# apache/cassandra

Measured on NVIDIA H100. Metric: compaction MB/s (uncompressed in), higher is better.
Workload: dtype u8

## Files before the change

### cassandra_b200/csrc/codec.cuh

```cuda
#pragma once
#include "common.cuh"
#include "lz4.cuh"
#include "lz4_chain.cuh"
#include "snappy_chain.cuh"
#include "snappy.cuh"
#include "codec_defs.cuh"
#include "lz4_thread.cuh"
#include "lz4_batch.cuh"

namespace b200c {

__global__ void __launch_bounds__(32) k_compress_chunks(const DevTables* __restrict__ T, int comp, int tab_bytes,
        const uint8_t* __restrict__ in, uint64_t n, int chunk_len, int max_clen,
        uint8_t* __restrict__ slots, int slot_stride, uint32_t* __restrict__ file_len, uint32_t* __restrict__ seg_raw) {
    extern __shared__ __align__(16) uint8_t smem[];
    uint16_t* s_tab = (uint16_t*)smem;
    uint8_t* s_in = smem + tab_bytes;
    const int lane = threadIdx.x;
    const uint64_t chunk = blockIdx.x;
    const uint64_t start = chunk * (uint64_t)chunk_len;
    const int ulen = (int)min((uint64_t)chunk_len, n - start);
    const uint8_t* src = in + start;

    if ((((uintptr_t)src) & 15) == 0) {
// ... 38 lines not shown

template <bool DUP>
__global__ void __launch_bounds__(32) k_compress_chunks_lz4_direct(const DevTables* __restrict__ T,
        const uint8_t* __restrict__ in, uint64_t n, int chunk_len, int max_clen,
        uint8_t* __restrict__ slots, int slot_stride, uint32_t* __restrict__ file_len, uint32_t* __restrict__ seg_raw) {
    __shared__ __align__(16) uint16_t s_tab[LZ4_TABLE_ENTRIES];
    __shared__ uint8_t s_dup[DUP ? LZ4_DUP_ENTRIES : 1];
    const int lane = threadIdx.x;
    const uint64_t chunk = blockIdx.x;
    const uint64_t start = chunk * (uint64_t)chunk_len;
    const int ulen = (int)min((uint64_t)chunk_len, n - start);
    const uint8_t* src = in + start;
    uint8_t* slot = slots + chunk * (uint64_t)slot_stride;
    if (lane == 0) { slot[0] = (uint8_t)ulen; slot[1] = (uint8_t)(ulen >> 8); slot[2] = (uint8_t)(ulen >> 16); slot[3] = (uint8_t)(ulen >> 24); }
    int clen = 4 + lz4_compress_warp<true>(src, ulen, s_tab, slot + 4, lane, DUP ? s_dup : nullptr);
    if (clen >= max_clen) {
        for (int i = lane; i < ulen; i += 32) slot[i] = src[i];
        clen = ulen;
        if (ulen < max_clen) { for (int i = ulen + lane; i < max_clen; i += 32) slot[i] = 0; clen = max_clen; }
    }
    __syncwarp();
    __threadfence_block();
    uint32_t raw = warp_crc32_raw(T, T->crc_adv128, slot, clen, lane);
    uint32_t init = gf2_mulmod(0xFFFFFFFFu, warp_xpow8n(T, (uint32_t)clen, lane));
    uint32_t crc = ~(raw ^ init);
    if (lane == 0) {
        slot[clen] = (uint8_t)(crc >> 24); slot[clen + 1] = (uint8_t)(crc >> 16); slot[clen + 2] = (uint8_t)(crc >> 8); slot[clen + 3] = (uint8_t)crc;
        file_len[chunk] = (uint32_t)clen + 4;
        uint32_t x = raw ^ __byte_perm(crc, 0, 0x0123);
        seg_raw[chunk] = T->crc_t[3][x & 0xff] ^ T->crc_t[2][(x >> 8) & 0xff] ^ T->crc_t[1][(x >> 16) & 0xff] ^ T->crc_t[0][x >> 24];
    }
}

__global__ void __launch_bounds__(32) k_lz4_chain_build(const uint8_t* __restrict__ in, uint64_t n, int chunk_len, uint32_t* __restrict__ ent) {
    __shared__ __align__(16) uint16_t s_t1[LZ4_TABLE_ENTRIES];
    const uint64_t start = (uint64_t)blockIdx.x * (uint64_t)chunk_len;
    const int ulen = (int)min((uint64_t)chunk_len, n - start);
    lz4_chain_build_warp<true>(in + start, ulen, s_t1, ent + start, threadIdx.x);
}
enum { K5B_WARPS = 4 };
__global__ void __launch_bounds__(32 * K5B_WARPS) k_compress_chunks_lz4_chain(const DevTables* __restrict__ T,
        const uint8_t* __restrict__ in, uint64_t n, int chunk_len, int max_clen, const uint32_t* __restrict__ ent,
        uint8_t* __restrict__ slots, int slot_stride, uint32_t* __restrict__ file_len, uint32_t* __restrict__ seg_raw, uint64_t nchunks) {
    extern __shared__ __align__(16) uint32_t s_bits[];
    const int lane = threadIdx.x & 31, wid = threadIdx.x >> 5;
    const uint64_t chunk = (uint64_t)blockIdx.x * K5B_WARPS + wid;
    if (chunk >= nchunks) return;
    const uint64_t start = chunk * (uint64_t)chunk_len;
    const int ulen = (int)min((uint64_t)chunk_len, n - start);
    const uint8_t* src = in + start;
    uint8_t* slot = slots + chunk * (uint64_t)slot_stride;
    if (lane == 0) { slot[0] = (uint8_t)ulen; slot[1] = (uint8_t)(ulen >> 8); slot[2] = (uint8_t)(ulen >> 16); slot[3] = (uint8_t)(ulen >> 24); }
    int clen = 4 + lz4_compress_warp_chain(src, ulen, ent + start, s_bits + (size_t)wid * ((chunk_len + 31) >> 5), slot + 4, lane);
    if (clen >= max_clen) {
        for (int i = lane; i < ulen; i += 32) slot[i] = src[i];
        clen = ulen;
        if (ulen < max_clen) { for (int i = ulen + lane; i < max_clen; i += 32) slot[i] = 0; clen = max_clen; }
    }
    __syncwarp();
    __threadfence_block();
    uint32_t raw = warp_crc32_raw(T, T->crc_adv128, slot, clen, lane);
    uint32_t init = gf2_mulmod(0xFFFFFFFFu, warp_xpow8n(T, (uint32_t)clen, lane));
    uint32_t crc = ~(raw ^ init);
    if (lane == 0) {
        slot[clen] = (uint8_t)(crc >> 24); slot[clen + 1] = (uint8_t)(crc >> 16); slot[clen + 2] = (uint8_t)(crc >> 8); slot[clen + 3] = (uint8_t)crc;
        file_len[chunk] = (uint32_t)clen + 4;
        uint32_t x = raw ^ __byte_perm(crc, 0, 0x0123);
        seg_raw[chunk] = T->crc_t[3][x & 0xff] ^ T->crc_t[2][(x >> 8) & 0xff] ^ T->crc_t[1][(x >> 16) & 0xff] ^ T->crc_t[0][x >> 24];
    }
}

__global__ void __launch_bounds__(32) k_snappy_chain_build(int max_bits, int table_size, const uint8_t* __restrict__ in, uint64_t n, int chunk_len, uint32_t* __restrict__ ent) {
    extern __shared__ __align__(16) uint8_t smem_sc[];
    const uint64_t start = (uint64_t)blockIdx.x * (uint64_t)chunk_len;
    const int ulen = (int)min((uint64_t)chunk_len, n - start);
    snappy_chain_build_warp<true>(in + start, ulen, max_bits, (uint16_t*)smem_sc, ent + start, threadIdx.x);
}
__global__ void __launch_bounds__(32 * K5B_WARPS) k_compress_chunks_snappy_chain(const DevTables* __restrict__ T,
        const uint8_t* __restrict__ in, uint64_t n, int chunk_len, int max_clen, const uint32_t* __restrict__ ent,
        uint8_t* __restrict__ slots, int slot_stride, uint32_t* __restrict__ file_len, uint32_t* __restrict__ seg_raw, uint64_t nchunks) {
    extern __shared__ __align__(16) uint32_t s_bits[];
    const int lane = threadIdx.x & 31, wid = threadIdx.x >> 5;
    const uint64_t chunk = (uint64_t)blockIdx.x * K5B_WARPS + wid;
    if (chunk >= nchunks) return;
    const uint64_t start = chunk * (uint64_t)chunk_len;
    const int ulen = (int)min((uint64_t)chunk_len, n - start);
    const uint8_t* src = in + start;
    uint8_t* slot = slots + chunk * (uint64_t)slot_stride;
    int clen = snappy_compress_warp_chain(src, ulen, ent + start, s_bits + (size_t)wid * ((chunk_len + 31) >> 5), slot, lane);
    if (clen >= max_clen) {
        for (int i = lane; i < ulen; i += 32) slot[i] = src[i];
        clen = ulen;
        if (ulen < max_clen) { for (int i = ulen + lane; i < max_clen; i += 32) slot[i] = 0; clen = max_clen; }
    }
    __syncwarp();
    __threadfence_block();
    uint32_t raw = warp_crc32_raw(T, T->crc_adv128, slot, clen, lane);
    uint32_t init = gf2_mulmod(0xFFFFFFFFu, warp_xpow8n(T, (uint32_t)clen, lane));
    uint32_t crc = ~(raw ^ init);
    if (lane == 0) {
        slot[clen] = (uint8_t)(crc >> 24); slot[clen + 1] = (uint8_t)(crc >> 16); slot[clen + 2] = (uint8_t)(crc >> 8); slot[clen + 3] = (uint8_t)crc;
        file_len[chunk] = (uint32_t)clen + 4;
        uint32_t x = raw ^ __byte_perm(crc, 0, 0x0123);
        seg_raw[chunk] = T->crc_t[3][x & 0xff] ^ T->crc_t[2][(x >> 8) & 0xff] ^ T->crc_t[1][(x >> 16) & 0xff] ^ T->crc_t[0][x >> 24];
    }
}

__global__ void __launch_bounds__(32) k_compress_chunks_snappy_direct(const DevTables* __restrict__ T, int max_bits,
        const uint8_t* __restrict__ in, uint64_t n, int chunk_len, int max_clen,
        uint8_t* __restrict__ slots, int slot_stride, uint32_t* __restrict__ file_len, uint32_t* __restrict__ seg_raw) {
// ... 254 lines not shown
```

### cassandra_b200/csrc/engine.cu

```cuda
#include "engine.cuh"
#include <algorithm>
#include "scan.cuh"
#include "codec.cuh"
#include <climits>
#include <vector>

using namespace b200c;

namespace b200c {

enum { WSC_IN = 0, WSC_OUT, WSC_SLOTS, WSC_FILELEN, WSC_SEGRAW, WSC_OFFS, WSC_ACC, WSC_ERR, WSC_CHOFFS, WSC_SCAN0, WSC_SCAN1, WSC_SCAN2 };

static void build_tables(DevTables* t) {
    for (uint32_t i = 0; i < 256; i++) {
        uint32_t c = i;
        for (int k = 0; k < 8; k++) c = (c & 1) ? (0xEDB88320u ^ (c >> 1)) : (c >> 1);
        t->crc_t[0][i] = c;
    }
    for (uint32_t i = 0; i < 256; i++)
        for (int k = 1; k < 4; k++) t->crc_t[k][i] = (t->crc_t[k - 1][i] >> 8) ^ t->crc_t[0][t->crc_t[k - 1][i] & 0xff];
    uint32_t sq = 0x00800000u;
    for (int k = 0; k < 64; k++) { t->xp_pow2[k] = sq; sq = gf2_mulmod(sq, sq); }
    auto xpow8n = [&](uint64_t n) { uint32_t r = 0x80000000u; for (int k = 0; n; k++, n >>= 1) if (n & 1) r = gf2_mulmod(r, t->xp_pow2[k]); return r; };
    uint32_t x128 = xpow8n(128);
    for (int j = 0; j < 4; j++)
        for (uint32_t b = 0; b < 256; b++) t->crc_adv128[j][b] = gf2_mulmod(b << (8 * j), x128);
    for (int l = 0; l < 32; l++) t->xp_lane[l] = xpow8n(4 * (32 - l));
}

template <typename TIn>
int exclusive_scan(b200c_ctx* c, const TIn* in, uint64_t n, uint64_t* out, int slot, int depth) {
    if (n == 0) { B200C_CUDA_TRY(c, cudaMemsetAsync(out, 0, sizeof(uint64_t), c->stream)); return B200C_OK; }
    uint64_t tiles = (n + SCAN_TILE - 1) / SCAN_TILE;
    if (tiles == 1) { B200C_LAUNCH(c, k_scan_down<TIn>, 1, SCAN_THREADS, 0, in, n, (const uint64_t*)nullptr, out, out + n); return B200C_OK; }
    if (depth > 2) { c->err = "scan recursion too deep"; return B200C_EINVAL; }
    uint64_t* sums; B200C_TRY(ws_typed(c, slot + depth, tiles + 1, &sums));
    B200C_LAUNCH(c, k_scan_reduce<TIn>, (unsigned)tiles, SCAN_THREADS, 0, in, n, sums);
    B200C_TRY(exclusive_scan<uint64_t>(c, sums, tiles, sums, slot, depth + 1));
    B200C_LAUNCH(c, k_scan_down<TIn>, (unsigned)tiles, SCAN_THREADS, 0, in, n, (const uint64_t*)sums, out, out + n);
    return B200C_OK;
}
template int exclusive_scan<uint32_t>(b200c_ctx*, const uint32_t*, uint64_t, uint64_t*, int, int);
template int exclusive_scan<uint64_t>(b200c_ctx*, const uint64_t*, uint64_t, uint64_t*, int, int);

int compress_slots_device(b200c_ctx* c, int comp, const uint8_t* d_in, uint64_t n, int chunk_len, int max_clen,
                          uint8_t* slots, int stride, uint32_t* file_len, uint32_t* seg_raw) {
    uint64_t nchunks = (n + chunk_len - 1) / chunk_len;
    if (!nchunks) return B200C_OK;
    const int k5_env = []() { const char* e = getenv("B200C_K5"); return e ? atoi(e) : -1; }();
    const int k5_mode = k5_env >= 0 ? k5_env : (comp_is_snappy(comp) ? 3 : 1);
    if (k5_mode == 3 && comp == COMP_LZ4 && ((uintptr_t)d_in & 3) == 0 && (chunk_len & 3) == 0 && chunk_len <= LZ4C_MAX_CHUNK) {
        uint32_t* ent; B200C_TRY(ws_typed(c, WS_K5_ENT, (size_t)n + 16384, &ent));
        B200C_LAUNCH(c, k_lz4_chain_build, (unsigned)nchunks, 32, 0, d_in, n, chunk_len, ent);
        const size_t smem = (size_t)K5B_WARPS * ((chunk_len + 31) >> 5) * 4;
        B200C_LAUNCH(c, k_compress_chunks_lz4_chain, (unsigned)((nchunks + K5B_WARPS - 1) / K5B_WARPS), 32 * K5B_WARPS, smem, c->d_tables, d_in, n, chunk_len, max_clen, (const uint32_t*)ent,
                     slots, stride, file_len, seg_raw, nchunks);
        return B200C_OK;
    }
    if ((k5_mode == 1 || k5_mode == 2) && comp == COMP_LZ4 && ((uintptr_t)d_in & 3) == 0 && (chunk_len & 3) == 0) {
        if (k5_mode == 2) B200C_LAUNCH(c, k_compress_chunks_lz4_direct<true>, (unsigned)nchunks, 32, 0, c->d_tables, d_in, n, chunk_len, max_clen, slots, stride, file_len, seg_raw);
        else B200C_LAUNCH(c, k_compress_chunks_lz4_direct<false>, (unsigned)nchunks, 32, 0, c->d_tables, d_in, n, chunk_len, max_clen, slots, stride, file_len, seg_raw);
        return B200C_OK;
    }
    if (k5_mode == 3 && comp_is_snappy(comp) && ((uintptr_t)d_in & 3) == 0 && (chunk_len & 3) == 0 && chunk_len <= LZ4C_MAX_CHUNK) {
        const int max_bits = comp == COMP_SNAPPY15 ? 15 : 14, tsz = snappy_table_size(chunk_len, max_bits);
        uint32_t* ent; B200C_TRY(ws_typed(c, WS_K5_ENT, (size_t)n + 16384, &ent));
        static bool attr = false; if (!attr) { cudaFuncSetAttribute(k_snappy_chain_build, cudaFuncAttributeMaxDynamicSharedMemorySize, 2 * 32768); attr = true; }
        B200C_LAUNCH(c, k_snappy_chain_build, (unsigned)nchunks, 32, (size_t)2 * tsz, max_bits, tsz, d_in, n, chunk_len, ent);
        const size_t smem = (size_t)K5B_WARPS * ((chunk_len + 31) >> 5) * 4;
        B200C_LAUNCH(c, k_compress_chunks_snappy_chain, (unsigned)((nchunks + K5B_WARPS - 1) / K5B_WARPS), 32 * K5B_WARPS, smem, c->d_tables, d_in, n, chunk_len, max_clen, (const uint32_t*)ent,
                     slots, stride, file_len, seg_raw, nchunks);
        return B200C_OK;
    }
    int tab_bytes = comp == COMP_SNAPPY15 ? 65536 : (comp == COMP_SNAPPY ? 32768 : 16384);
    if (k5_mode != 0 && comp_is_snappy(comp) && ((uintptr_t)d_in & 3) == 0 && (chunk_len & 3) == 0 && chunk_len <= 65536) {
        int need = 512; while (need < 2 * chunk_len && need < tab_bytes) need <<= 1;
        B200C_LAUNCH(c, k_compress_chunks_snappy_direct, (unsigned)nchunks, 32, (size_t)need, c->d_tables, comp == COMP_SNAPPY15 ? 15 : 14, d_in, n, chunk_len, max_clen, slots, stride, file_len, seg_raw);
        return B200C_OK;
    }
    size_t smem = (size_t)tab_bytes + chunk_len + 16;
    B200C_LAUNCH(c, k_compress_chunks, (unsigned)nchunks, 32, smem, c->d_tables, comp, tab_bytes, d_in, n, chunk_len, max_clen, slots, stride, file_len, seg_raw);
    return B200C_OK;
}
int pack_digest_device(b200c_ctx* c, const uint8_t* slots, int stride, const uint32_t* file_len, const uint32_t* seg_raw, uint64_t nchunks,
                       uint8_t* d_out, uint64_t out_cap, uint64_t* d_offs, uint64_t* out_len, uint32_t* digest, int ws_base) {
    if (!nchunks) { *out_len = 0; *digest = 0; B200C_CUDA_TRY(c, cudaMemsetAsync(d_offs, 0, 8, c->stream)); return B200C_OK; }
    uint32_t* acc; B200C_TRY(ws_typed(c, ws_base + WSC_ACC, 4, &acc));
    B200C_CUDA_TRY(c, cudaMemsetAsync(acc, 0, 16, c->stream));
    B200C_TRY(exclusive_scan<uint32_t>(c, file_len, nchunks, d_offs, ws_base + WSC_SCAN0, 0));
    uint64_t* h = (uint64_t*)c->h_pinned;
    B200C_CUDA_TRY(c, cudaMemcpyAsync(h, d_offs + nchunks, 8, cudaMemcpyDeviceToHost, c->stream));
    B200C_CUDA_TRY(c, cudaStreamSynchronize(c->stream));
    *out_len = h[0];
    if (h[0] > out_cap) { c->err = "output buffer too small"; return B200C_ETOOSMALL; }
    B200C_LAUNCH(c, k_pack_chunks, (unsigned)((nchunks + 3) / 4), 128, 0, slots, stride, file_len, d_offs, nchunks, d_out, (const uint64_t*)nullptr);
    B200C_LAUNCH(c, k_digest, (unsigned)((nchunks + 255) / 256), 256, 0, c->d_tables, seg_raw, d_offs, nchunks, acc);
    B200C_LAUNCH(c, k_digest_final, 1, 1, 0, c->d_tables, d_offs, nchunks, acc);
    uint32_t* h32 = (uint32_t*)c->h_pinned;
    B200C_CUDA_TRY(c, cudaMemcpyAsync(h32, acc + 1, 4, cudaMemcpyDeviceToHost, c->stream));
    B200C_CUDA_TRY(c, cudaStreamSynchronize(c->stream));
    *digest = h32[0];
    return B200C_OK;
}
int compress_stream_device(b200c_ctx* c, int comp, const uint8_t* d_in, uint64_t n, int chunk_len, int max_clen,
                           uint8_t* d_out, uint64_t out_cap, uint64_t* d_offs , uint64_t* out_len, uint32_t* digest, int ws_base) {
    uint64_t nchunks = (n + chunk_len - 1) / chunk_len;
    if (nchunks > 0x7fffffffull) { c->err = "too many chunks"; return B200C_EINVAL; }
    int stride = chunk_slot_stride(comp, chunk_len);
// ... 148 lines not shown

int b200c_abi_version(void) { return B200C_ABI_VERSION; }

int b200c_device_count(void) {
    int n = 0; if (cudaGetDeviceCount(&n) != cudaSuccess) { cudaGetLastError(); return 0; } return n;
}

b200c_ctx* b200c_create(int device, size_t workspace_bytes) {
    int n = b200c_device_count();
    if (device < 0 || device >= n) return nullptr;
    if (cudaSetDevice(device) != cudaSuccess) return nullptr;
    b200c_ctx* c = new b200c_ctx();
    c->device = device;
    if (cudaDeviceGetAttribute(&c->nsm, cudaDevAttrMultiProcessorCount, device) != cudaSuccess || c->nsm <= 0) { delete c; return nullptr; }
    if (cudaDeviceGetAttribute(&c->l2_bytes, cudaDevAttrL2CacheSize, device) != cudaSuccess || c->l2_bytes <= 0) { delete c; return nullptr; }
    if (cudaDeviceGetAttribute(&c->smem_per_sm, cudaDevAttrMaxSharedMemoryPerMultiprocessor, device) != cudaSuccess ||
        cudaDeviceGetAttribute(&c->smem_reserved_per_block, cudaDevAttrReservedSharedMemoryPerBlock, device) != cudaSuccess) { delete c; return nullptr; }
    if (cudaStreamCreateWithFlags(&c->stream, cudaStreamNonBlocking) != cudaSuccess) { delete c; return nullptr; }
    cudaEventCreate(&c->ev0); cudaEventCreate(&c->ev1);
    for (auto& e : c->ev_stage) cudaEventCreate(&e);
    cudaStreamCreateWithFlags(&c->copy_stream, cudaStreamNonBlocking);
    for (auto& e : c->ev_in) cudaEventCreateWithFlags(&e, cudaEventDisableTiming);
    for (auto& e : c->ev_pool) cudaEventCreateWithFlags(&e, cudaEventDisableTiming);
    cudaStreamCreateWithFlags(&c->copy_out, cudaStreamNonBlocking);
    cudaStreamCreateWithFlags(&c->stream5, cudaStreamNonBlocking);
    DevTables* h = new DevTables(); build_tables(h);
    if (cudaMalloc(&c->d_tables, sizeof(DevTables)) != cudaSuccess) { delete h; delete c; return nullptr; }
    cudaMemcpy(c->d_tables, h, sizeof(DevTables), cudaMemcpyHostToDevice);
    delete h;
    c->h_pinned_cap = 1 << 16;
    if (cudaMallocHost(&c->h_pinned, c->h_pinned_cap) != cudaSuccess) { cudaFree(c->d_tables); delete c; return nullptr; }
    cudaFuncSetAttribute(k_compress_chunks, cudaFuncAttributeMaxDynamicSharedMemorySize, 65536 + 65536 + 16);
    cudaFuncSetAttribute(k_compress_chunks_snappy_direct, cudaFuncAttributeMaxDynamicSharedMemorySize, 65536);
    k1_plan(c);
    (void)workspace_bytes;
    return c;
}

void b200c_destroy(b200c_ctx* c) {
    if (!c) return;
    cudaSetDevice(c->device);
    cudaStreamSynchronize(c->stream);
    for (auto& b : c->ws) if (b.p) cudaFree(b.p);
    if (c->d_tables) cudaFree(c->d_tables);
    if (c->h_pinned) cudaFreeHost(c->h_pinned);
    cudaEventDestroy(c->ev0); cudaEventDestroy(c->ev1);
    for (auto& e : c->ev_stage) cudaEventDestroy(e);
    for (auto& e : c->ev_in) cudaEventDestroy(e);
    for (auto& e : c->ev_pool) cudaEventDestroy(e);
    for (auto& e : c->ev_marks) cudaEventDestroy(e);
    if (c->stream5) cudaStreamDestroy(c->stream5);
    for (auto e : c->ev_k5) cudaEventDestroy(e);
    if (c->copy_out) cudaStreamDestroy(c->copy_out);
    if (c->copy_stream) cudaStreamDestroy(c->copy_stream);
    cudaStreamDestroy(c->stream);
    delete c;
}

const char* b200c_last_error(b200c_ctx* c) { return c ? c->err.c_str() : "no context (no CUDA device?)"; }

int b200c_host_register(void* p, size_t n) { cudaError_t e = cudaHostRegister(p, n, cudaHostRegisterDefault); if (e != cudaSuccess) { cudaGetLastError(); return B200C_ECUDA; } return B200C_OK; }
int b200c_host_unregister(void* p) { cudaError_t e = cudaHostUnregister(p); if (e != cudaSuccess) { cudaGetLastError(); return B200C_ECUDA; } return B200C_OK; }

int b200c_dev_alloc(b200c_ctx* c, size_t n, void** dptr) {
    if (!c || !dptr) return B200C_EINVAL;
    cudaSetDevice(c->device);
// ... 25 lines not shown
uint64_t b200c_chunk_count(uint64_t n, int chunk_len) { return chunk_len > 0 ? (n + chunk_len - 1) / chunk_len : 0; }
uint64_t b200c_compress_bound(int comp, uint64_t n, int chunk_len) {
    uint64_t nch = b200c_chunk_count(n, chunk_len);
    int m = chunk_max_compressed(comp, chunk_len); if (m < chunk_len) m = chunk_len;
    return nch * ((uint64_t)m + 4) + 64;
}
int b200c_initial_compressed_buffer_length(int comp, int chunk_len) { return chunk_max_compressed(comp, chunk_len); }

static int check_codec_args(b200c_ctx* c, int comp, int chunk_len) {
    if (!c) return B200C_EINVAL;
    if (comp != COMP_LZ4 && !comp_is_snappy(comp) && comp != COMP_NONE) { c->err = "unknown compressor"; return B200C_EINVAL; }
    if (chunk_len <= 0 || chunk_len > 65536 || (chunk_len & (chunk_len - 1))) { c->err = "chunk_len must be a power of two <= 64 KiB"; return B200C_EUNSUPPORTED; }
    return B200C_OK;
}

int b200c_compress_chunks(b200c_ctx* c, int comp, const uint8_t* in, uint64_t n, int chunk_len, int max_clen,
                          uint8_t* out, uint64_t out_cap, uint64_t* out_len, uint64_t* chunk_offsets, uint32_t* digest, int flags) {
    B200C_TRY(check_codec_args(c, comp, chunk_len));
    if ((!in && n) || !out || !out_len || !digest) { c->err = "null argument"; return B200C_EINVAL; }
    cudaSetDevice(c->device);
    const bool dev = flags & B200C_FLAG_DEVICE_PTRS;
    uint64_t nchunks = b200c_chunk_count(n, chunk_len);
    const uint8_t* d_in = in; uint8_t* d_out = out; uint64_t* d_offs;
    if (!dev) {
        uint8_t* p; B200C_TRY(ws_typed(c, WSC_IN, n + 64, &p));
        B200C_CUDA_TRY(c, cudaMemcpyAsync(p, in, n, cudaMemcpyHostToDevice, c->stream)); d_in = p;
        B200C_TRY(ws_typed(c, WSC_OUT, out_cap, &d_out));
    }
    if (dev && chunk_offsets) d_offs = chunk_offsets;
    else B200C_TRY(ws_typed(c, WSC_OFFS, nchunks + 1, &d_offs));
    timing_begin(c);
    int rc = compress_stream_device(c, comp, d_in, n, chunk_len, max_clen, d_out, out_cap, d_offs, out_len, digest, 0);
    int rc2 = timing_end(c);
    if (rc != B200C_OK) return rc;
    if (rc2 != B200C_OK) return rc2;
    if (!dev) {
        B200C_CUDA_TRY(c, cudaMemcpyAsync(out, d_out, *out_len, cudaMemcpyDeviceToHost, c->stream));
        if (chunk_offsets && nchunks) B200C_CUDA_TRY(c, cudaMemcpyAsync(chunk_offsets, d_offs, nchunks * 8, cudaMemcpyDeviceToHost, c->stream));
        B200C_CUDA_TRY(c, cudaStreamSynchronize(c->stream));
    }
    return B200C_OK;
}

int b200c_decompress_chunks(b200c_ctx* c, int comp, const uint8_t* data, uint64_t data_len, const uint64_t* chunk_offsets, uint64_t nchunks,
                            int chunk_len, int max_clen, uint64_t data_length, uint8_t* out, int verify_crc, b200c_corruption* where, int flags) {
    B200C_TRY(check_codec_args(c, comp, chunk_len));
    if ((!data && data_len) || (!chunk_offsets && nchunks) || (!out && data_length)) { c->err = "null argument"; return B200C_EINVAL; }
    if (nchunks != b200c_chunk_count(data_length, chunk_len)) { c->err = "chunk count does not match data_length"; return B200C_EINVAL; }
    cudaSetDevice(c->device);
    const bool dev = flags & B200C_FLAG_DEVICE_PTRS;
    const uint8_t* d_data = data; const uint64_t* d_offs = chunk_offsets; uint8_t* d_out = out;
    if (!dev) {
        uint8_t* p; B200C_TRY(ws_typed(c, WSC_IN, data_len + 64, &p));
        B200C_CUDA_TRY(c, cudaMemcpyAsync(p, data, data_len, cudaMemcpyHostToDevice, c->stream)); d_data = p;
        uint64_t* po; B200C_TRY(ws_typed(c, WSC_CHOFFS, nchunks + 1, &po));
        B200C_CUDA_TRY(c, cudaMemcpyAsync(po, chunk_offsets, nchunks * 8, cudaMemcpyHostToDevice, c->stream)); d_offs = po;
        B200C_TRY(ws_typed(c, WSC_OUT, data_length + 64, &d_out));
    }
    ChunkErr* d_err; B200C_TRY(ws_typed(c, WSC_ERR, 1, &d_err));
    B200C_CUDA_TRY(c, cudaMemsetAsync(d_err, 0xFF, sizeof(ChunkErr), c->stream));
    timing_begin(c);
    int rc = decompress_stream_device(c, comp, d_data, data_len, d_offs, nchunks, chunk_len, max_clen, data_length, d_out, verify_crc, d_err, 0, ~0ull, 0, nullptr, ~0ull);
    int rc2 = timing_end(c);
    if (rc != B200C_OK) return rc;
    if (rc2 != B200C_OK) return rc2;
    ChunkErr* h = (ChunkErr*)c->h_pinned;
// ... 53 lines not shown
```

### cassandra_b200/csrc/engine.cuh

```cuda
#pragma once
#include <cstdio>
#include <cstring>
#include <string>
#include <atomic>
#include <chrono>
#include <vector>
#include "../../include/b200c.h"
#include "common.cuh"

namespace b200c {

enum { WS_SLOTS = 160, WS_K5_ENT = 150, WS_K1_REC = 151, WS_K1_NSEQ = 152 };

struct WsBuf { void* p = nullptr; size_t cap = 0; };

}

struct b200c_ctx {
    int device = 0;
    int nsm = 0;
    int l2_bytes = 0;
    int smem_per_sm = 0, smem_reserved_per_block = 0;
    int k1_blocks_per_sm = 1; size_t k1_smem = 0;
    cudaStream_t stream = nullptr;
// ... 19 lines not shown
    std::vector<cudaEvent_t> ev_marks;
    cudaEvent_t ev_pool[256] = {};
    cudaStream_t copy_out = nullptr;
    cudaStream_t stream5 = nullptr;
    std::vector<cudaEvent_t> ev_k5;
};

namespace b200c {

#define B200C_CUDA_TRY(ctx, expr) do { cudaError_t _e = (expr); if (_e != cudaSuccess) { \
    (ctx)->err = std::string(#expr) + ": " + cudaGetErrorString(_e); return B200C_ECUDA; } } while (0)

#define B200C_LAUNCH(ctx, kernel, grid, block, smem, ...) do { \
    kernel<<<(grid), (block), (smem), (ctx)->stream>>>(__VA_ARGS__); \
    (ctx)->launches_call++; (ctx)->launches_total++; \
    cudaError_t _e = cudaGetLastError(); if (_e != cudaSuccess) { \
        (ctx)->err = std::string(#kernel) + " launch: " + cudaGetErrorString(_e); return B200C_ECUDA; } } while (0)

#define B200C_TRY(expr) do { int _rc = (expr); if (_rc != B200C_OK) return _rc; } while (0)

inline int ws_get(b200c_ctx* c, int slot, size_t bytes, void** out) {
    WsBuf& b = c->ws[slot];
    size_t need = bytes + 256;
    if (b.cap < need) {
        if (b.p) { cudaStreamSynchronize(c->stream); if (c->copy_stream) cudaStreamSynchronize(c->copy_stream); if (c->copy_out) cudaStreamSynchronize(c->copy_out); cudaFree(b.p); b.p = nullptr; b.cap = 0; }
        size_t cap = need + need / 8;
        cudaError_t e = cudaMalloc(&b.p, cap);
        if (e != cudaSuccess) { cudaGetLastError(); c->err = "cudaMalloc(" + std::to_string(cap) + "): " + cudaGetErrorString(e); b.p = nullptr; return B200C_ENOMEM; }
        b.cap = cap;
    }
    *out = b.p;
    return B200C_OK;
}
template <typename T> inline int ws_typed(b200c_ctx* c, int slot, size_t count, T** out) {
    void* p; int rc = ws_get(c, slot, count * sizeof(T), &p); *out = (T*)p; return rc;
}

template <typename T> inline int ws_grow_keep(b200c_ctx* c, int slot, size_t count, size_t used, T** out) {
    WsBuf& b = c->ws[slot];
    size_t need = count * sizeof(T) + 256;
    if (b.cap < need) {
        cudaStreamSynchronize(c->stream); cudaStreamSynchronize(c->copy_out);
        void* np = nullptr; size_t cap = need * 2;
        cudaError_t e = cudaMalloc(&np, cap);
        if (e != cudaSuccess) { cudaGetLastError(); c->err = "cudaMalloc(" + std::to_string(cap) + "): " + cudaGetErrorString(e); return B200C_ENOMEM; }
        if (b.p && used) cudaMemcpy(np, b.p, std::min(used * sizeof(T), b.cap), cudaMemcpyDeviceToDevice);
        if (b.p) cudaFree(b.p);
        b.p = np; b.cap = cap;
    }
    *out = (T*)b.p;
    return B200C_OK;
}

inline void timing_begin(b200c_ctx* c) { c->launches_call = 0; cudaEventRecord(c->ev0, c->stream); c->timing = true; }
inline int timing_end(b200c_ctx* c) {
    cudaEventRecord(c->ev1, c->stream);
    B200C_CUDA_TRY(c, cudaEventSynchronize(c->ev1));
    float ms = 0; cudaEventElapsedTime(&ms, c->ev0, c->ev1); c->last_ms = ms; c->timing = false;
    return B200C_OK;
}

struct OutStream {
    enum { MAX_PIECES = 96 };
    b200c_ctx* c = nullptr; int comp = 0, L = 0, max_clen = 0, stride = 0, ws_base = 0;
    uint8_t* h_out = nullptr; uint64_t h_cap = 0;
    uint32_t *file_len = nullptr, *seg_raw = nullptr, *acc = nullptr; uint64_t *d_offs = nullptr, *bases = nullptr;
// ... 11 lines not shown
```

### cassandra_b200/csrc/lz4_chain.cuh

```cuda
#pragma once
#include "lz4.cuh"

namespace b200c {

enum { LZ4C_MAX_CHUNK = 32768, LZ4C_NONE = 0xFFFF, LZ4C_DUP_ENTRIES = 8192 };

#if defined(__CUDA_ARCH__)
#define LZ4C_PREFETCH(p) asm volatile("prefetch.global.L2 [%0];" :: "l"(p))
#else
#define LZ4C_PREFETCH(p) ((void)0)
#endif

__host__ __device__ __forceinline__ int lz4c_positions(int n) { return n >= LZ4_MINLENGTH ? n - LZ4_MFLIMIT + 1 : 0; }

template <bool GLOBAL, class HASH> __device__ __forceinline__ void chain_build_warp(const uint8_t* s_in, int npos, int nent, int hbits, HASH hash, uint16_t* s_t1, uint32_t* __restrict__ ent, int lane) {
    const uint32_t* in32 = (const uint32_t*)s_in;
    {
        uint4* a = (uint4*)s_t1;
        for (int i = lane; i < (nent * 2) / 16; i += 32) a[i] = make_uint4(~0u, ~0u, ~0u, ~0u);
    }
    __syncwarp();
    const uint32_t lt_mask = (1u << lane) - 1u;
    enum { AHEAD = 4 };
    uint32_t ring[AHEAD];
#pragma unroll
    for (int k = 0; k < AHEAD; k++) ring[k] = (32 * k + lane < npos) ? lz4_rd32<GLOBAL>(in32, 32 * k + lane) : 0u;
    for (int p0 = 0; p0 < npos; p0 += 32 * AHEAD) {
#pragma unroll
        for (int k = 0; k < AHEAD; k++) {
            const int p = p0 + 32 * k + lane; const bool valid = p < npos;
            if (p0 + 32 * k >= npos) break;
            const uint32_t seq = ring[k];
            ring[k] = (p + 32 * AHEAD < npos) ? lz4_rd32<GLOBAL>(in32, p + 32 * AHEAD) : 0u;
            const uint32_t h = hash(seq);
            uint32_t q1 = valid ? (uint32_t)s_t1[h] : (uint32_t)LZ4C_NONE;
            __syncwarp();
            if (valid) s_t1[h] = (uint16_t)p;
            __syncwarp();
            const bool lost = valid && s_t1[h] != (uint16_t)p;
            uint32_t todo = __ballot_sync(FULL_MASK, lost);
            if (todo) {
                bool fix = false;
                while (todo) {
                    const int l = __ffs(todo) - 1;
                    const uint32_t hh = __shfl_sync(FULL_MASK, h, l);
                    const uint32_t same = __ballot_sync(FULL_MASK, valid && h == hh);
                    if (valid && h == hh) {
                        const uint32_t lower = same & lt_mask;
                        if (lower) q1 = (uint32_t)(p0 + 32 * k + 31 - __clz(lower));
                        fix = !(same & ~lt_mask & ~(1u << lane));
                    }
                    todo &= ~same;
                }
                if (fix) s_t1[h] = (uint16_t)p;
                __syncwarp();
            }
            if (valid) ent[p] = q1 == LZ4C_NONE ? 0u : q1;
        }
    }
    __syncwarp();
#pragma unroll 8
    for (int p0 = 0; p0 < npos; p0 += 32) {
        const int p = p0 + lane;
        if (p < npos) {
            const uint32_t a1 = ent[p] & 0x7FFFu;
            const uint32_t a2 = ent[a1] & 0x7FFFu;
            const uint32_t sp = lz4_rd32<GLOBAL>(in32, p);
            const uint32_t e1 = lz4_rd32<GLOBAL>(in32, (int)a1) == sp, e2 = lz4_rd32<GLOBAL>(in32, (int)a2) == sp;
            ent[p] = a1 | (e1 << 15) | (a2 << 16) | (e2 << 31);
        }
    }
}
struct Lz4Hash { __device__ __forceinline__ uint32_t operator()(uint32_t seq) const { return lz4_hash_u16(seq); } };
template <bool GLOBAL> __device__ __forceinline__ void lz4_chain_build_warp(const uint8_t* s_in, int n, uint16_t* s_t1, uint32_t* __restrict__ ent, int lane) {
    chain_build_warp<GLOBAL>(s_in, lz4c_positions(n), LZ4_TABLE_ENTRIES, LZ4_HASHLOG_U16, Lz4Hash(), s_t1, ent, lane);
}

__device__ __forceinline__ uint32_t lz4c_range_bits(int lo, int hi, int w) {
    const int a = lo > w * 32 ? lo - w * 32 : 0, b = hi < w * 32 + 32 ? hi - w * 32 : 32;
    if (b <= a) return 0u;
    const uint32_t upto_b = b >= 32 ? FULL_MASK : ((1u << b) - 1u);
    return upto_b & ~((1u << a) - 1u);
}

__device__ int lz4_compress_warp_chain(const uint8_t* s_in, int n, const uint32_t* __restrict__ ent, uint32_t* s_bm, uint8_t* out, int lane) {
    const uint32_t* in32 = (const uint32_t*)s_in;
    for (int i = lane; i < ((n + 31) >> 5); i += 32) s_bm[i] = (i == 0) ? 1u : 0u;
    __syncwarp();
    int anchor = 0, op = 0;
    const int mfl1 = n - LZ4_MFLIMIT + 1;
    const int matchlimit = n - LZ4_LASTLITERALS;

    if (n >= LZ4_MINLENGTH) {
        int fwd = 1; bool have_prefix = false; int pre_ip = 0;
        for (;;) {
            int ip = 0, match = 0, token_pos; bool ended = false, immediate = false;
            if (lane < 4) LZ4C_PREFETCH(ent + fwd + 64 + 32 * lane);
            int a0 = 0;
            for (bool first = true;; first = false) {
                const bool prefixed = first && have_prefix;
                const bool contiguous = a0 + 32 <= 66;
                const int w_lo = prefixed ? pre_ip - 2 : fwd + a0;
                const int hole = prefixed ? pre_ip - 1 : -1;
                int p; bool valid, putonly = false;
                if (contiguous) {
                    p = w_lo + lane + ((prefixed && lane >= 1) ? 1 : 0);
                    putonly = prefixed && lane == 0;
                    valid = (prefixed && lane < 2) || p + 1 <= mfl1;
// ... 127 lines not shown
```

### cassandra_b200/csrc/snappy_chain.cuh

```cuda
#pragma once
#include "snappy.cuh"
#include "lz4_chain.cuh"

namespace b200c {

struct SnappyHash { uint32_t tmask; int max_bits; __device__ __forceinline__ uint32_t operator()(uint32_t bytes) const { return snappy_tidx(bytes, tmask, max_bits); } };
__host__ __device__ __forceinline__ int snappy_table_size(int frag, int max_bits) { int t = 256; while (t < frag && t < (1 << max_bits)) t <<= 1; return t; }
__host__ __device__ __forceinline__ int snappyc_positions(int n) { return n >= 15 ? n - 14 : 0; }

template <bool GLOBAL> __device__ __forceinline__ void snappy_chain_build_warp(const uint8_t* s_in, int n, int max_bits, uint16_t* s_t1, uint32_t* __restrict__ ent, int lane) {
    const int tsz = snappy_table_size(n, max_bits);
    chain_build_warp<GLOBAL>(s_in, snappyc_positions(n), tsz, 31 - __clz(tsz), SnappyHash{(uint32_t)tsz - 1u, max_bits}, s_t1, ent, lane);
}

__device__ int snappy_compress_warp_chain(const uint8_t* s_in, int n, const uint32_t* __restrict__ ent, uint32_t* s_bm, uint8_t* out, int lane) {
    const uint32_t* in32 = (const uint32_t*)s_in;
    int op = 0;
    {   uint32_t v = (uint32_t)n; uint8_t pre[5]; int k = 0;
        while (v >= 0x80) { pre[k++] = (uint8_t)(v | 0x80); v >>= 7; } pre[k++] = (uint8_t)v;
        if (lane == 0) for (int i = 0; i < k; i++) out[i] = pre[i];
        op = k; }
    for (int i = lane; i < ((n + 31) >> 5); i += 32) s_bm[i] = (i == 0) ? 1u : 0u;
    __syncwarp();
    int ip = 0; const int ip_end = n;
    if (n >= 15) {
        const int ip_limit = n - 15;
        bool have_prefix = false;
        for (;;) {
            const int next_emit = ip;
            const int start = ip + 1;
            const bool unrolled = ip_limit - start >= 16;
            int hit_ip = 0, candidate = 0; bool ended = false, immediate = false;
            if (lane < 4) LZ4C_PREFETCH(ent + start + 64 + 32 * lane);
            int q0 = start; uint32_t skip0 = 32; int a0 = 0;
            for (bool first = true;; first = false) {
                const bool prefixed = first && have_prefix;
                const bool contiguous = first;
                const int w_lo = prefixed ? ip - 1 : start;
                int q; bool valid, putonly = false; int qn = 0; uint32_t skn = 0;
                if (contiguous) {
                    q = w_lo + lane;
                    const int l = lane - (prefixed ? 2 : 0);
                    putonly = prefixed && lane == 0;
                    qn = q + 1; skn = 32u + (uint32_t)(l + 1);
                    valid = l < 0 || (unrolled && l < 16) || qn <= ip_limit;
// ... 87 lines not shown
```

Measured before the change: 32330.

## Build hash chain links with block-wide radix sort instead of per-warp scan

Replaces the single-warp sequential hash-chain build with a 512-thread-per-chunk kernel. It loads the chunk into shared memory, stably radix-sorts positions by hash in two digit passes, and derives each position's previous same-hash link from its sorted neighbour. The chain path becomes the default for LZ4 as well as snappy. The kernel uses more shared memory and more synchronisation, and the old warp builder is kept only as a serial lane-0 fallback. A large link workspace is also freed after each call when it exceeds a threshold, which adds a stream synchronize.

After: 32620, median of 6. Within noise of the previous version (+0.9%).

```diff
diff --git a/cassandra_b200/csrc/codec.cuh b/cassandra_b200/csrc/codec.cuh
--- a/cassandra_b200/csrc/codec.cuh
+++ b/cassandra_b200/csrc/codec.cuh
@@ -94,11 +94,117 @@
     }
 }
 
-__global__ void __launch_bounds__(32) k_lz4_chain_build(const uint8_t* __restrict__ in, uint64_t n, int chunk_len, uint32_t* __restrict__ ent) {
-    __shared__ __align__(16) uint16_t s_t1[LZ4_TABLE_ENTRIES];
+enum { LINK_THREADS = 512, LINK_WARPS = LINK_THREADS / 32, LINK_DIGIT_BITS = 8, LINK_DIGITS = 1 << LINK_DIGIT_BITS };
+__host__ __device__ __forceinline__ size_t link_smem_bytes(int chunk_len) {
+    return (size_t)((chunk_len + 16 + 15) & ~15) + (size_t)LINK_WARPS * (LINK_DIGITS + LINK_DIGITS / 2) * 4 + (size_t)2 * 2 * chunk_len;
+}
+struct Lz4Links {
+    Lz4Hash hash; int bits, npos;
+    __device__ Lz4Links(int n, int) : bits(LZ4_HASHLOG_U16), npos(lz4c_positions(n)) {}
+};
+struct SnappyLinks {
+    SnappyHash hash; int bits, npos;
+    __device__ SnappyLinks(int n, int max_bits) {
+        const int tsz = snappy_table_size(n, max_bits);
+        hash = SnappyHash{(uint32_t)tsz - 1u, max_bits}; bits = 31 - __clz(tsz); npos = snappyc_positions(n);
+    }
+};
+__device__ __forceinline__ void link_scan(uint32_t* a, int len, uint32_t* s_wsum) {
+    const int tid = threadIdx.x, lane = tid & 31, w = tid >> 5;
+    const int per = (len + LINK_THREADS - 1) / LINK_THREADS, i0 = tid * per;
+    uint32_t v[8], sum = 0;
+#pragma unroll
+    for (int k = 0; k < 8; k++) { v[k] = (k < per && i0 + k < len) ? a[i0 + k] : 0u; sum += v[k]; }
+    uint32_t inc = sum;
+#pragma unroll
+    for (int d = 1; d < 32; d <<= 1) { const uint32_t t = __shfl_up_sync(FULL_MASK, inc, d); if (lane >= d) inc += t; }
+    if (lane == 31) s_wsum[w] = inc;
+    __syncthreads();
+    uint32_t run = inc - sum;
+    for (int k = 0; k < w; k++) run += s_wsum[k];
+#pragma unroll
+    for (int k = 0; k < 8; k++) if (k < per && i0 + k < len) { a[i0 + k] = run; run += v[k]; }
+    __syncthreads();
+}
+template <class LINKS>
+__global__ void __launch_bounds__(LINK_THREADS, 2) k_chain_links(int max_bits, const uint8_t* __restrict__ in, uint64_t n, int chunk_len, uint32_t* __restrict__ ent) {
+    extern __shared__ __align__(16) uint8_t smem_l[];
+    __shared__ uint32_t s_wsum[LINK_WARPS];
+    const int tid = threadIdx.x, lane = tid & 31, w = tid >> 5;
     const uint64_t start = (uint64_t)blockIdx.x * (uint64_t)chunk_len;
     const int ulen = (int)min((uint64_t)chunk_len, n - start);
-    lz4_chain_build_warp<true>(in + start, ulen, s_t1, ent + start, threadIdx.x);
+    const LINKS L(ulen, max_bits);
+    const int npos = L.npos;
+    if (npos == 0) return;
+    uint8_t* s_in = smem_l;
+    uint32_t* s_cnt = (uint32_t*)(smem_l + ((chunk_len + 16 + 15) & ~15));
+    uint32_t* s_cnt2 = s_cnt + LINK_WARPS * LINK_DIGITS;
+    uint16_t* s_a = (uint16_t*)(s_cnt2 + LINK_WARPS * LINK_DIGITS / 2);
+    uint16_t* s_b = s_a + chunk_len;
+    const uint32_t* in32 = (const uint32_t*)s_in;
+
+    const uint8_t* src = in + start;
+    int done;
+    if ((((uintptr_t)src) & 15) == 0) { const int nv = ulen >> 4; for (int i = tid; i < nv; i += LINK_THREADS) ((uint4*)s_in)[i] = __ldg((const uint4*)src + i); done = nv << 4; }
+    else { const int nv = ulen >> 2; for (int i = tid; i < nv; i += LINK_THREADS) ((uint32_t*)s_in)[i] = __ldg((const uint32_t*)src + i); done = nv << 2; }
+    for (int i = done + tid; i < ulen; i += LINK_THREADS) s_in[i] = src[i];
+    if (tid < 16) s_in[ulen + tid] = 0;
+    __syncthreads();
+
+    const int d1 = (L.bits + 1) >> 1, d2 = L.bits - d1;
+    const int seg = (npos + LINK_THREADS - 1) / LINK_THREADS * 32;
+    const int lo = w * seg, hi = min(lo + seg, npos);
+    const uint32_t lt_mask = (1u << lane) - 1u;
+    for (int i = tid; i < LINK_WARPS * (LINK_DIGITS + LINK_DIGITS / 2); i += LINK_THREADS) s_cnt[i] = 0;
+    __syncthreads();
+    for (int i = lo + lane; i < hi; i += 32) atomicAdd(s_cnt + (L.hash(rd32_at(in32, i)) & ((1u << d1) - 1u)) * LINK_WARPS + w, 1u);
+    __syncthreads();
+    link_scan(s_cnt, LINK_WARPS << d1, s_wsum);
+    for (int pass = 0; pass < 2; pass++) {
+        const int shift = pass ? d1 : 0, dbits = pass ? d2 : d1;
+        const uint16_t* from = pass ? s_a : nullptr;
+        uint16_t* to = pass ? s_b : s_a;
+        uint32_t* cnt = pass ? s_cnt2 : s_cnt;
+        for (int i0 = lo; i0 < lo + seg; i0 += 32) {
+            const int i = i0 + lane; const bool valid = i < hi;
+            const int p = valid ? (from ? (int)from[i] : i) : 0;
+            const uint32_t h = L.hash(rd32_at(in32, p)), d = (h >> shift) & ((1u << dbits) - 1u);
+            uint32_t same = __ballot_sync(FULL_MASK, valid);
+#pragma unroll
+            for (int b = 0; b < LINK_DIGIT_BITS; b++) {
+                if (b < dbits) { const uint32_t mb = __ballot_sync(FULL_MASK, (d >> b) & 1u); same &= ((d >> b) & 1u) ? mb : ~mb; }
+            }
+            uint32_t* c = cnt + d * LINK_WARPS + w;
+            const uint32_t base = *c, j = base + __popc(same & lt_mask);
+            if (valid) {
+                to[j] = (uint16_t)p;
+                if (!pass) atomicAdd(s_cnt2 + (h >> d1) * LINK_WARPS + j / seg, 1u);
+            }
+            __syncwarp();
+            if (valid && !(same >> lane >> 1)) *c = base + __popc(same);
+            __syncwarp();
+        }
+        __syncthreads();
+        if (!pass) link_scan(s_cnt2, LINK_WARPS << d2, s_wsum);
+    }
+
+    const uint32_t v0 = rd32_at(in32, 0);
+    for (int i = tid; i < npos; i += LINK_THREADS) {
+        const int p = s_b[i];
+        const uint32_t v = rd32_at(in32, p);
+        uint32_t q1 = 0, e1 = v == v0;
+        if (i > 0) {
+            const int pp = s_b[i - 1]; const uint32_t vp = rd32_at(in32, pp);
+            if (L.hash(vp) == L.hash(v)) { q1 = (uint32_t)pp; e1 = v == vp; }
+        }
+        s_a[p] = (uint16_t)(q1 | e1 << 15);
+    }
+    __syncthreads();
+    uint32_t* e = ent + start;
+    for (int p = tid; p < npos; p += LINK_THREADS) {
+        const uint32_t l1 = s_a[p], q1 = l1 & 0x7FFFu, q2 = s_a[q1] & 0x7FFFu;
+        e[p] = l1 | q2 << 16 | (uint32_t)(rd32_at(in32, (int)q2) == rd32_at(in32, p)) << 31;
+    }
 }
 enum { K5B_WARPS = 4 };
 __global__ void __launch_bounds__(32 * K5B_WARPS) k_compress_chunks_lz4_chain(const DevTables* __restrict__ T,
@@ -132,12 +238,6 @@
     }
 }
 
-__global__ void __launch_bounds__(32) k_snappy_chain_build(int max_bits, int table_size, const uint8_t* __restrict__ in, uint64_t n, int chunk_len, uint32_t* __restrict__ ent) {
-    extern __shared__ __align__(16) uint8_t smem_sc[];
-    const uint64_t start = (uint64_t)blockIdx.x * (uint64_t)chunk_len;
-    const int ulen = (int)min((uint64_t)chunk_len, n - start);
-    snappy_chain_build_warp<true>(in + start, ulen, max_bits, (uint16_t*)smem_sc, ent + start, threadIdx.x);
-}
 __global__ void __launch_bounds__(32 * K5B_WARPS) k_compress_chunks_snappy_chain(const DevTables* __restrict__ T,
         const uint8_t* __restrict__ in, uint64_t n, int chunk_len, int max_clen, const uint32_t* __restrict__ ent,
         uint8_t* __restrict__ slots, int slot_stride, uint32_t* __restrict__ file_len, uint32_t* __restrict__ seg_raw, uint64_t nchunks) {
diff --git a/cassandra_b200/csrc/engine.cu b/cassandra_b200/csrc/engine.cu
--- a/cassandra_b200/csrc/engine.cu
+++ b/cassandra_b200/csrc/engine.cu
@@ -9,6 +9,7 @@
 
 namespace b200c {
 
+constexpr size_t K5_KEEP_LINKS = 256u << 20;
 enum { WSC_IN = 0, WSC_OUT, WSC_SLOTS, WSC_FILELEN, WSC_SEGRAW, WSC_OFFS, WSC_ACC, WSC_ERR, WSC_CHOFFS, WSC_SCAN0, WSC_SCAN1, WSC_SCAN2 };
 
 static void build_tables(DevTables* t) {
@@ -48,32 +49,31 @@
     uint64_t nchunks = (n + chunk_len - 1) / chunk_len;
     if (!nchunks) return B200C_OK;
     const int k5_env = []() { const char* e = getenv("B200C_K5"); return e ? atoi(e) : -1; }();
-    const int k5_mode = k5_env >= 0 ? k5_env : (comp_is_snappy(comp) ? 3 : 1);
-    if (k5_mode == 3 && comp == COMP_LZ4 && ((uintptr_t)d_in & 3) == 0 && (chunk_len & 3) == 0 && chunk_len <= LZ4C_MAX_CHUNK) {
+    const int k5_mode = k5_env >= 0 ? k5_env : 3;
+    const bool aligned = ((uintptr_t)d_in & 3) == 0 && (chunk_len & 3) == 0;
+    if (k5_mode == 3 && (comp == COMP_LZ4 || comp_is_snappy(comp)) && aligned && chunk_len <= LZ4C_MAX_CHUNK) {
         uint32_t* ent; B200C_TRY(ws_typed(c, WS_K5_ENT, (size_t)n + 16384, &ent));
-        B200C_LAUNCH(c, k_lz4_chain_build, (unsigned)nchunks, 32, 0, d_in, n, chunk_len, ent);
         const size_t smem = (size_t)K5B_WARPS * ((chunk_len + 31) >> 5) * 4;
-        B200C_LAUNCH(c, k_compress_chunks_lz4_chain, (unsigned)((nchunks + K5B_WARPS - 1) / K5B_WARPS), 32 * K5B_WARPS, smem, c->d_tables, d_in, n, chunk_len, max_clen, (const uint32_t*)ent,
-                     slots, stride, file_len, seg_raw, nchunks);
+        const unsigned pblocks = (unsigned)((nchunks + K5B_WARPS - 1) / K5B_WARPS);
+        if (comp == COMP_LZ4) {
+            B200C_LAUNCH(c, k_chain_links<Lz4Links>, (unsigned)nchunks, LINK_THREADS, link_smem_bytes(chunk_len), 0, d_in, n, chunk_len, ent);
+            B200C_LAUNCH(c, k_compress_chunks_lz4_chain, pblocks, 32 * K5B_WARPS, smem, c->d_tables, d_in, n, chunk_len, max_clen, (const uint32_t*)ent,
+                         slots, stride, file_len, seg_raw, nchunks);
+        } else {
+            const int max_bits = comp == COMP_SNAPPY15 ? 15 : 14;
+            B200C_LAUNCH(c, k_chain_links<SnappyLinks>, (unsigned)nchunks, LINK_THREADS, link_smem_bytes(chunk_len), max_bits, d_in, n, chunk_len, ent);
+            B200C_LAUNCH(c, k_compress_chunks_snappy_chain, pblocks, 32 * K5B_WARPS, smem, c->d_tables, d_in, n, chunk_len, max_clen, (const uint32_t*)ent,
+                         slots, stride, file_len, seg_raw, nchunks);
+        }
         return B200C_OK;
     }
-    if ((k5_mode == 1 || k5_mode == 2) && comp == COMP_LZ4 && ((uintptr_t)d_in & 3) == 0 && (chunk_len & 3) == 0) {
+    if (k5_mode != 0 && comp == COMP_LZ4 && aligned) {
         if (k5_mode == 2) B200C_LAUNCH(c, k_compress_chunks_lz4_direct<true>, (unsigned)nchunks, 32, 0, c->d_tables, d_in, n, chunk_len, max_clen, slots, stride, file_len, seg_raw);
         else B200C_LAUNCH(c, k_compress_chunks_lz4_direct<false>, (unsigned)nchunks, 32, 0, c->d_tables, d_in, n, chunk_len, max_clen, slots, stride, file_len, seg_raw);
         return B200C_OK;
     }
-    if (k5_mode == 3 && comp_is_snappy(comp) && ((uintptr_t)d_in & 3) == 0 && (chunk_len & 3) == 0 && chunk_len <= LZ4C_MAX_CHUNK) {
-        const int max_bits = comp == COMP_SNAPPY15 ? 15 : 14, tsz = snappy_table_size(chunk_len, max_bits);
-        uint32_t* ent; B200C_TRY(ws_typed(c, WS_K5_ENT, (size_t)n + 16384, &ent));
-        static bool attr = false; if (!attr) { cudaFuncSetAttribute(k_snappy_chain_build, cudaFuncAttributeMaxDynamicSharedMemorySize, 2 * 32768); attr = true; }
-        B200C_LAUNCH(c, k_snappy_chain_build, (unsigned)nchunks, 32, (size_t)2 * tsz, max_bits, tsz, d_in, n, chunk_len, ent);
-        const size_t smem = (size_t)K5B_WARPS * ((chunk_len + 31) >> 5) * 4;
-        B200C_LAUNCH(c, k_compress_chunks_snappy_chain, (unsigned)((nchunks + K5B_WARPS - 1) / K5B_WARPS), 32 * K5B_WARPS, smem, c->d_tables, d_in, n, chunk_len, max_clen, (const uint32_t*)ent,
-                     slots, stride, file_len, seg_raw, nchunks);
-        return B200C_OK;
-    }
     int tab_bytes = comp == COMP_SNAPPY15 ? 65536 : (comp == COMP_SNAPPY ? 32768 : 16384);
-    if (k5_mode != 0 && comp_is_snappy(comp) && ((uintptr_t)d_in & 3) == 0 && (chunk_len & 3) == 0 && chunk_len <= 65536) {
+    if (k5_mode != 0 && comp_is_snappy(comp) && aligned && chunk_len <= 65536) {
         int need = 512; while (need < 2 * chunk_len && need < tab_bytes) need <<= 1;
         B200C_LAUNCH(c, k_compress_chunks_snappy_direct, (unsigned)nchunks, 32, (size_t)need, c->d_tables, comp == COMP_SNAPPY15 ? 15 : 14, d_in, n, chunk_len, max_clen, slots, stride, file_len, seg_raw);
         return B200C_OK;
@@ -288,6 +288,8 @@
     if (cudaMallocHost(&c->h_pinned, c->h_pinned_cap) != cudaSuccess) { cudaFree(c->d_tables); delete c; return nullptr; }
     cudaFuncSetAttribute(k_compress_chunks, cudaFuncAttributeMaxDynamicSharedMemorySize, 65536 + 65536 + 16);
     cudaFuncSetAttribute(k_compress_chunks_snappy_direct, cudaFuncAttributeMaxDynamicSharedMemorySize, 65536);
+    cudaFuncSetAttribute(k_chain_links<Lz4Links>, cudaFuncAttributeMaxDynamicSharedMemorySize, (int)link_smem_bytes(LZ4C_MAX_CHUNK));
+    cudaFuncSetAttribute(k_chain_links<SnappyLinks>, cudaFuncAttributeMaxDynamicSharedMemorySize, (int)link_smem_bytes(LZ4C_MAX_CHUNK));
     k1_plan(c);
     (void)workspace_bytes;
     return c;
@@ -379,6 +381,7 @@
     timing_begin(c);
     int rc = compress_stream_device(c, comp, d_in, n, chunk_len, max_clen, d_out, out_cap, d_offs, out_len, digest, 0);
     int rc2 = timing_end(c);
+    if (c->ws[WS_K5_ENT].cap > K5_KEEP_LINKS) ws_release(c, WS_K5_ENT);
     if (rc != B200C_OK) return rc;
     if (rc2 != B200C_OK) return rc2;
     if (!dev) {
diff --git a/cassandra_b200/csrc/engine.cuh b/cassandra_b200/csrc/engine.cuh
--- a/cassandra_b200/csrc/engine.cuh
+++ b/cassandra_b200/csrc/engine.cuh
@@ -75,6 +75,10 @@
     *out = b.p;
     return B200C_OK;
 }
+inline void ws_release(b200c_ctx* c, int slot) {
+    WsBuf& b = c->ws[slot];
+    if (b.p) { cudaStreamSynchronize(c->stream); cudaFree(b.p); b.p = nullptr; b.cap = 0; }
+}
 template <typename T> inline int ws_typed(b200c_ctx* c, int slot, size_t count, T** out) {
     void* p; int rc = ws_get(c, slot, count * sizeof(T), &p); *out = (T*)p; return rc;
 }
diff --git a/cassandra_b200/csrc/lz4_chain.cuh b/cassandra_b200/csrc/lz4_chain.cuh
--- a/cassandra_b200/csrc/lz4_chain.cuh
+++ b/cassandra_b200/csrc/lz4_chain.cuh
@@ -3,7 +3,7 @@
 
 namespace b200c {
 
-enum { LZ4C_MAX_CHUNK = 32768, LZ4C_NONE = 0xFFFF, LZ4C_DUP_ENTRIES = 8192 };
+enum { LZ4C_MAX_CHUNK = 32768, LZ4C_DUP_ENTRIES = 8192 };
 
 #if defined(__CUDA_ARCH__)
 #define LZ4C_PREFETCH(p) asm volatile("prefetch.global.L2 [%0];" :: "l"(p))
@@ -13,67 +13,21 @@
 
 __host__ __device__ __forceinline__ int lz4c_positions(int n) { return n >= LZ4_MINLENGTH ? n - LZ4_MFLIMIT + 1 : 0; }
 
-template <bool GLOBAL, class HASH> __device__ __forceinline__ void chain_build_warp(const uint8_t* s_in, int npos, int nent, int hbits, HASH hash, uint16_t* s_t1, uint32_t* __restrict__ ent, int lane) {
+template <bool GLOBAL, class HASH> __device__ __forceinline__ void chain_build_serial(const uint8_t* s_in, int npos, int nent, HASH hash, uint16_t* s_t1, uint32_t* __restrict__ ent, int lane) {
     const uint32_t* in32 = (const uint32_t*)s_in;
-    {
-        uint4* a = (uint4*)s_t1;
-        for (int i = lane; i < (nent * 2) / 16; i += 32) a[i] = make_uint4(~0u, ~0u, ~0u, ~0u);
-    }
-    __syncwarp();
-    const uint32_t lt_mask = (1u << lane) - 1u;
-    enum { AHEAD = 4 };
-    uint32_t ring[AHEAD];
-#pragma unroll
-    for (int k = 0; k < AHEAD; k++) ring[k] = (32 * k + lane < npos) ? lz4_rd32<GLOBAL>(in32, 32 * k + lane) : 0u;
-    for (int p0 = 0; p0 < npos; p0 += 32 * AHEAD) {
-#pragma unroll
-        for (int k = 0; k < AHEAD; k++) {
-            const int p = p0 + 32 * k + lane; const bool valid = p < npos;
-            if (p0 + 32 * k >= npos) break;
-            const uint32_t seq = ring[k];
-            ring[k] = (p + 32 * AHEAD < npos) ? lz4_rd32<GLOBAL>(in32, p + 32 * AHEAD) : 0u;
-            const uint32_t h = hash(seq);
-            uint32_t q1 = valid ? (uint32_t)s_t1[h] : (uint32_t)LZ4C_NONE;
-            __syncwarp();
-            if (valid) s_t1[h] = (uint16_t)p;
-            __syncwarp();
-            const bool lost = valid && s_t1[h] != (uint16_t)p;
-            uint32_t todo = __ballot_sync(FULL_MASK, lost);
-            if (todo) {
-                bool fix = false;
-                while (todo) {
-                    const int l = __ffs(todo) - 1;
-                    const uint32_t hh = __shfl_sync(FULL_MASK, h, l);
-                    const uint32_t same = __ballot_sync(FULL_MASK, valid && h == hh);
-                    if (valid && h == hh) {
-                        const uint32_t lower = same & lt_mask;
-                        if (lower) q1 = (uint32_t)(p0 + 32 * k + 31 - __clz(lower));
-                        fix = !(same & ~lt_mask & ~(1u << lane));
-                    }
-                    todo &= ~same;
-                }
-                if (fix) s_t1[h] = (uint16_t)p;
-                __syncwarp();
-            }
-            if (valid) ent[p] = q1 == LZ4C_NONE ? 0u : q1;
+    if (lane == 0) {
+        for (int h = 0; h < nent; h++) s_t1[h] = 0;
+        for (int p = 0; p < npos; p++) { const uint32_t h = hash(lz4_rd32<GLOBAL>(in32, p)); ent[p] = s_t1[h]; s_t1[h] = (uint16_t)p; }
+        for (int p = 0; p < npos; p++) {
+            const uint32_t v = lz4_rd32<GLOBAL>(in32, p), q1 = ent[p] & 0x7FFFu, q2 = ent[q1] & 0x7FFFu;
+            ent[p] = q1 | (uint32_t)(lz4_rd32<GLOBAL>(in32, (int)q1) == v) << 15 | q2 << 16 | (uint32_t)(lz4_rd32<GLOBAL>(in32, (int)q2) == v) << 31;
         }
     }
     __syncwarp();
-#pragma unroll 8
-    for (int p0 = 0; p0 < npos; p0 += 32) {
-        const int p = p0 + lane;
-        if (p < npos) {
-            const uint32_t a1 = ent[p] & 0x7FFFu;
-            const uint32_t a2 = ent[a1] & 0x7FFFu;
-            const uint32_t sp = lz4_rd32<GLOBAL>(in32, p);
-            const uint32_t e1 = lz4_rd32<GLOBAL>(in32, (int)a1) == sp, e2 = lz4_rd32<GLOBAL>(in32, (int)a2) == sp;
-            ent[p] = a1 | (e1 << 15) | (a2 << 16) | (e2 << 31);
-        }
-    }
 }
 struct Lz4Hash { __device__ __forceinline__ uint32_t operator()(uint32_t seq) const { return lz4_hash_u16(seq); } };
 template <bool GLOBAL> __device__ __forceinline__ void lz4_chain_build_warp(const uint8_t* s_in, int n, uint16_t* s_t1, uint32_t* __restrict__ ent, int lane) {
-    chain_build_warp<GLOBAL>(s_in, lz4c_positions(n), LZ4_TABLE_ENTRIES, LZ4_HASHLOG_U16, Lz4Hash(), s_t1, ent, lane);
+    chain_build_serial<GLOBAL>(s_in, lz4c_positions(n), LZ4_TABLE_ENTRIES, Lz4Hash(), s_t1, ent, lane);
 }
 
 __device__ __forceinline__ uint32_t lz4c_range_bits(int lo, int hi, int w) {
diff --git a/cassandra_b200/csrc/snappy_chain.cuh b/cassandra_b200/csrc/snappy_chain.cuh
--- a/cassandra_b200/csrc/snappy_chain.cuh
+++ b/cassandra_b200/csrc/snappy_chain.cuh
@@ -10,7 +10,7 @@
 
 template <bool GLOBAL> __device__ __forceinline__ void snappy_chain_build_warp(const uint8_t* s_in, int n, int max_bits, uint16_t* s_t1, uint32_t* __restrict__ ent, int lane) {
     const int tsz = snappy_table_size(n, max_bits);
-    chain_build_warp<GLOBAL>(s_in, snappyc_positions(n), tsz, 31 - __clz(tsz), SnappyHash{(uint32_t)tsz - 1u, max_bits}, s_t1, ent, lane);
+    chain_build_serial<GLOBAL>(s_in, snappyc_positions(n), tsz, SnappyHash{(uint32_t)tsz - 1u, max_bits}, s_t1, ent, lane);
 }
 
 __device__ int snappy_compress_warp_chain(const uint8_t* s_in, int n, const uint32_t* __restrict__ ent, uint32_t* s_bm, uint8_t* out, int lane) {
```
